# Komputerowe-Projektowanie-Lekow/pmarlo

Hardware: AMD Instinct MI355X
Metric: frames/sec featurize->TICA->k-means->T-matrix, 1Mx64 synth; ITS rel-err (higher is better)
Workload: dtype f64; 1 GPU; synthetic 1000000 frames x 64 f32 features per GPU (AR(1) latents), TICA->10, k=500 (10 Lloyd iterations), lag=10, row-normalised T; frames_per_gpu=1000000, features=64, tica_dim=10, k=500, lag=10, kmeans_iters=10, parallelism=shards1

## Files before the change

include/msmhip.h:

```cpp
#ifndef MSMHIP_H
#define MSMHIP_H

#include <stddef.h>
#include <stdint.h>

#ifdef __cplusplus
extern "C" {
#endif

typedef struct msm_ctx msm_ctx;
typedef struct msm_event msm_event;
typedef struct msm_graph msm_graph;

typedef enum {
    MSM_OK = 0,
    MSM_ERR_INVALID = 1,
    MSM_ERR_HIP = 2,
    MSM_ERR_NOMEM = 3,
    MSM_ERR_UNSUPPORTED = 4,
    MSM_ERR_NOCONV = 5
} msm_status;

typedef enum { MSM_F32 = 0, MSM_F64 = 1 } msm_dtype;

// ... 100 lines not shown
msm_status msm_lagged_moments_onesided(msm_ctx* ctx, const void* d_x, msm_dtype dtype, int64_t n, int F,
                                       int64_t ld, const int64_t* h_seg_start, const int64_t* h_seg_stop,
                                       int n_seg, int lag, const double* d_shift, int assume_finite,
                                       double* d_moments);

msm_status msm_onesided_tica_eigenvalues(msm_ctx* ctx, const double* d_moments, int F, double clip,
                                         double* d_eigvals);

msm_status msm_moments_from_lagged(msm_ctx* ctx, const void* d_x, msm_dtype dtype, int64_t n, int F, int64_t ld,
                                   const int64_t* h_seg_start, const int64_t* h_seg_stop, int n_seg, int lag,
                                   const double* d_shift, const double* d_moments, double* d_sums);

msm_status msm_tica_solve(msm_ctx* ctx, const double* d_moments, const double* d_scale, int F,
                          double epsilon, int kinetic_map, double* d_eigvals, double* d_coeffs,
                          double* d_mean, int* d_rank);

msm_status msm_project(msm_ctx* ctx, const void* d_x, msm_dtype dtype, int64_t n, int F, int64_t ld,
                       const double* d_mu, const double* d_inv_sigma, const double* d_mean2,
                       const double* d_w, int d, int64_t ldw, double* d_y, int64_t ldy, double* d_absmax);

msm_status msm_project_finite(msm_ctx* ctx, const void* d_x, msm_dtype dtype, int64_t n, int F, int64_t ld,
                              const double* d_mu, const double* d_inv_sigma, const double* d_mean2,
                              const double* d_w, int d, int64_t ldw, double* d_y, int64_t ldy, double* d_absmax);

msm_status msm_eigh(msm_ctx* ctx, const double* d_a, int n, double* d_w, double* d_v, int* d_sweeps);

msm_status msm_autocorr_lagscan(msm_ctx* ctx, const void* d_x, msm_dtype dtype, int64_t n, int F, int64_t ld,
                                const int64_t* h_seg_start, const int64_t* h_seg_stop, int n_seg,
                                const int32_t* h_lags, int n_lag, double var_floor, double* d_value,
                                int32_t* d_nvalid);
// ... 212 lines not shown
```

pmarlo_amd/_lib.py:

```python

from __future__ import annotations

import ctypes as C
from pathlib import Path

__all__ = ["lib", "load", "LIB_PATH", "check", "MsmError", "DECLARED_SYMBOLS"]

LIB_PATH = Path(__file__).resolve().parent / "csrc" / "libmsmhip.so"

MSM_OK, MSM_ERR_INVALID, MSM_ERR_HIP, MSM_ERR_NOMEM, MSM_ERR_UNSUPPORTED, MSM_ERR_NOCONV = range(6)
MSM_F32, MSM_F64 = 0, 1
SUPERPOSE_TILE_FRAMES, SUPERPOSE_TILE_FLOATS, SUPERPOSE_LDS_ATOMS, SUPERPOSE_NARROW_SEL = 64, 12288, 4096, 64
REP_MAX_D, REP_GROUP_CHUNK, REP_TILE_I, REP_TILE_J = 256, 1024, 128, 64
REP_FLAG_NONFINITE, REP_FLAG_NEGATIVE, REP_FLAG_NONPOSITIVE_SUM = 1, 2, 4
REP_SCORE_CENTROID, REP_SCORE_MEDOID = 0, 1
REP_SELECT_SMALLEST, REP_SELECT_DIVERSE = 0, 1
SIL_SEG_LEN, SIL_TILE_I = 1024, 128
COMBINE_MAX_SEG, FLUX_LDS_MAX_N = 32, 127


class MsmError(RuntimeError):
    """A HIP-side failure reported through the C ABI."""


# ... 34 lines not shown
    "msm_hbond_presence": (_i32, [_vp, _vp, _i64, _i32, _vp, _i32, C.c_float, C.c_float, _vp]),
    "msm_dssp": (_i32, [_vp, _vp, _i64, _i32, _vp, _vp, _vp, _i32, _vp]),
    "msm_superpose": (_i32, [_vp, _vp, _i64, _i32, _vp, _i32, _vp, _vp, _vp]),
    "msm_count_transitions": (_i32, [_vp, _vp, _i64, _vp, _vp, _i32, _i32, _i32, _i32, _vp, _vp]),
    "msm_count_transitions_weighted": (
        _i32, [_vp, _vp, _vp, _i64, _vp, _vp, _i32, _i32, _i32, _i32, _vp, _vp]),
    "msm_count_transitions_lagscan": (_i32, [_vp, _vp, _i64, _vp, _vp, _i32, _vp, _i32, _i32, _vp, _vp]),
    "msm_state_counts": (_i32, [_vp, _vp, _i64, _i32, _vp]),
    "msm_column_moments_partial": (_i32, [_vp, _vp, _i32, _i64, _i32, _i64, _vp, _vp, _vp]),
    "msm_moments_finalize": (_i32, [_vp, _vp, _vp, _i32, _i32, _vp, _vp, _vp]),
    "msm_column_moments": (_i32, [_vp, _vp, _i32, _i64, _i32, _i64, _i32, _vp, _vp, _vp]),
    "msm_column_minmax": (_i32, [_vp, _vp, _i32, _i64, _i32, _i64, _vp, _vp, _vp]),
    "msm_standardise_params": (_i32, [_vp, _vp, _vp, _i32, _f64, _i32, _vp, _vp, _vp]),
    "msm_lagged_moments": (_i32, [_vp, _vp, _i32, _i64, _i32, _i64, _vp, _vp, _i32, _i32, _vp, _i32, _vp]),
    "msm_tica_solve": (_i32, [_vp, _vp, _vp, _i32, _f64, _i32, _vp, _vp, _vp, _vp]),
    "msm_lagged_moments_reversible": (_i32, [_vp, _vp, _i32, _i64, _i32, _i64, _vp, _vp, _i32, _i32, _vp, _i32, _vp]),
    "msm_lagged_moments_onesided": (_i32, [_vp, _vp, _i32, _i64, _i32, _i64, _vp, _vp, _i32, _i32, _vp, _i32, _vp]),
    "msm_onesided_tica_eigenvalues": (_i32, [_vp, _vp, _i32, _f64, _vp]),
    "msm_moments_from_lagged": (_i32, [_vp, _vp, _i32, _i64, _i32, _i64, _vp, _vp, _i32, _i32, _vp, _vp, _vp]),
    "msm_project": (_i32, [_vp, _vp, _i32, _i64, _i32, _i64, _vp, _vp, _vp, _vp, _i32, _i64, _vp, _i64, _vp]),
    "msm_project_finite": (_i32, [_vp, _vp, _i32, _i64, _i32, _i64, _vp, _vp, _vp, _vp, _i32, _i64, _vp, _i64, _vp]),
    "msm_eigh": (_i32, [_vp, _vp, _i32, _vp, _vp, _vp]),
    "msm_autocorr_lagscan": (_i32, [_vp, _vp, _i32, _i64, _i32, _i64, _vp, _vp, _i32, _vp, _i32, _f64, _vp, _vp]),
    "msm_hstack_f64": (_i32, [_vp, _vp, _i32, _i32, _i64, _vp, _i32, _i32, _i64, _i64, _vp]),
    "msm_kmeans_assign": (_i32, [_vp, _vp, _i32, _i64, _i32, _i64, _vp, _i32, _vp, _vp, _vp, _vp]),
    "msm_kmeans_fit": (_i32, [_vp, _vp, _i32, _i64, _i32, _i64, _vp, _vp, _i32, C.c_uint64, _i32, _i32, _f64, _vp, _vp]),
    "msm_kmeans_fit_begin": (
        _i32, [_vp, _vp, _i32, _i64, _i32, _i64, _vp, _vp, _i32, C.c_uint64, _i32, _f64, _f64, _vp, _vp, _i32]),
    "msm_kmeans_accumulate": (_i32, [_vp, _vp, _i32, _i64, _i32, _i64, _vp, _i32, _vp, _vp, _vp, _vp, _vp]),
    "msm_kmeans_update": (_i32, [_vp, _vp, _vp, _i32, _i32, _vp, _vp, _i32]),
# ... 121 lines not shown
```

pmarlo_amd/csrc/eig.hip:

```cpp
#include "common.h"
#include "wave.h"

__device__ __forceinline__ unsigned long long stamp_clock() {
    unsigned long long t;
    asm volatile("s_memtime %0\n\ts_waitcnt lgkmcnt(0)" : "=s"(t)::"memory");
    return t;
}
#define STAMP_ADD(slot, last) do { const unsigned long long t__ = stamp_clock(); slot += t__ - last; last = t__; } while (0)
#ifdef MSM_JACOBI_STAMPS
__device__ unsigned long long g_jacobi_stamps[8];
#define JSTAMP(i) STAMP_ADD(acc__[i], last__)
#define JSTAMP_INIT unsigned long long acc__[8] = {0, 0, 0, 0, 0, 0, 0, 0}; unsigned long long last__ = stamp_clock();
#define JSTAMP_FLUSH if (threadIdx.x == 0) { for (int i__ = 0; i__ < 8; ++i__) g_jacobi_stamps[i__] += acc__[i__]; }
#else
#define JSTAMP(i)
#define JSTAMP_INIT
#define JSTAMP_FLUSH
#endif
#ifdef MSM_TRI_STAMPS
__device__ unsigned long long g_tri_stamps[24];
#define TSTAMP(i) do { if (threadIdx.x == 0) STAMP_ADD(g_tri_stamps[i], tlast__); } while (0)
#define TSTAMP_INIT unsigned long long tlast__ = 0; if (threadIdx.x == 0) tlast__ = stamp_clock();
#define KSTAMP(i) do { if (threadIdx.x == 0) STAMP_ADD(g_tri_stamps[i], klast__); } while (0)
#define KSTAMP_INIT unsigned long long klast__ = 0; if (threadIdx.x == 0) klast__ = stamp_clock();
// ... 678 lines not shown
        for (int t = 0; t < 8; ++t)
            if (lane == sub + 8 * t && lane < n) ts->inv[lane] = nr_rsqrt(m[t]);
    }
    __syncthreads();
    if (what == 1 && in) {
#pragma unroll
        for (int t = 0; t < 8; ++t) {
            const int i = sub + 8 * t;
            if (i < n) W[lane * ld + i] = m[t] * ts->inv[i];
        }
    }
    __syncthreads();
    return true;
}

__device__ __forceinline__ bool tridiag_eigh(double* A, double* Q, double* X, int n, int ld, TriShared* ts, double orth_tol) {
    const int tid = threadIdx.x, nt = blockDim.x, lane = tid & 63, wave = tid >> 6;
    if (n == 1) {
        if (tid == 0) { ts->lam[0] = A[0]; A[0] = 1.0; }
        __syncthreads();
        return true;
    }
    if (ld != kTriLd) return false;
    TSTAMP_INIT
    if (tid == 0) ts->bad = 0;
    __syncthreads();
    TSTAMP(0);
    householder_phase(A, Q, n, ts);
    TSTAMP(1);
    __syncthreads();
    TSTAMP(2);
    {
// ... 14 lines not shown
            else ts->de[lane] = make_double2(8.0, 0.0);
            if (lane < 8) ts->de[kTriMax + lane] = make_double2(8.0, 0.0);
            if (lane == 0) {
                if (!(an < 1e300)) ts->bad = 1;
                ts->scale = sc;
                const double bn = fmax(fabs(gl), fabs(gu));
                const double pad = 4.0 * n * 2.220446049250313e-16 * bn + 1e-290;
                ts->gl = gl - pad;
                ts->gu = gu + pad;
            }
        }
    }
    __syncthreads();
    TSTAMP(3);
    if (ts->bad) return false;
    if (tid < 8 * kTriMax && wave * 8 < n) {
        const int i = tid >> 3, t = tid & 7;
        const int nblocks = (n + 7) >> 3;
        double lo = ts->gl, hi = ts->gu;
        const double frac = (double)(t + 1) * (1.0 / 9.0);
        for (int it = 0; it < 20; ++it) {
            const double x = fma(hi - lo, frac, lo);
            const int c = sturm_count(ts, nblocks, x);
            double nlo = c <= i ? x : lo, nhi = c > i ? x : hi;
            lo = row8_reduce(nlo, hw_max_f64);
            hi = row8_reduce(nhi, hw_min_f64);
        }
        if (i < n && t == 0) ts->lam[i] = 0.5 * (lo + hi);
    }
    __syncthreads();
    TSTAMP(4);
    const double tiny = 1e-290;
    double* Xc = X + (lane < n ? lane : 0);
    double* Ac = A + (lane < n ? lane : 0);
    const double lamb = ts->lam[lane < n ? lane : 0];
    if (wave == 0 && lane < n) {
        double q = ts->de[0].x - lamb;
        Xc[0] = q;
        for (int j0 = 1; j0 < n; j0 += 8) {
            double2 r[8];
#pragma unroll
            for (int u = 0; u < 8; ++u) r[u] = ts->de[j0 + u];
#pragma unroll
            for (int u = 0; u < 8; ++u) {
                if (j0 + u < n) {
                    if (fabs(q) < tiny) q = -tiny;
                    q = fma(-r[u].y, nr_rcp(q), r[u].x - lamb);
                    Xc[(j0 + u) * ld] = q;
                }
            }
        }
    } else if (wave == 1 && lane < n) {
        double r = ts->de[n - 1].x - lamb;
        if (fabs(r) < tiny) r = -tiny;
        double ir = nr_rcp(r);
        Ac[(n - 1) * ld] = ir;
        for (int j0 = n - 2; j0 >= 0; j0 -= 8) {
            double dj[8], e2[8];
#pragma unroll
            for (int u = 0; u < 8; ++u) {
                const int j = j0 - u >= 0 ? j0 - u : 0;
                dj[u] = ts->de[j].x;
                e2[u] = ts->de[j + 1].y;
            }
#pragma unroll
            for (int u = 0; u < 8; ++u) {
                if (j0 - u >= 0) {
                    r = fma(-e2[u], ir, dj[u] - lamb);
                    if (fabs(r) < tiny) r = -tiny;
                    ir = nr_rcp(r);
                    Ac[(j0 - u) * ld] = ir;
                }
            }
        }
    }
    __syncthreads();
    int kk = n - 1;
    if (wave < 2 && lane < n) {
        double gbest = fabs(Xc[(n - 1) * ld]);
        for (int j0 = n - 2; j0 >= 0; j0 -= 8) {
            double g[8];
#pragma unroll
            for (int u = 0; u < 8; ++u) {
                const int j = j0 - u >= 0 ? j0 - u : 0;
                g[u] = fabs(fma(-ts->de[j + 1].y, Ac[(j + 1) * ld], Xc[j * ld]));
            }
#pragma unroll
            for (int u = 0; u < 8; ++u)
                if (j0 - u >= 0 && g[u] <= gbest) { gbest = g[u]; kk = j0 - u; }
        }
    }
    __syncthreads();
    if (wave == 0 && lane < n) {
        double z = 1.0, nrm2 = 1.0;
        for (int j0 = n - 2; j0 >= 0; j0 -= 8) {
            double f[8];
#pragma unroll
            for (int u = 0; u < 8; ++u) {
                const int j = j0 - u >= 0 ? j0 - u : 0;
                double qq = Xc[j * ld];
                if (fabs(qq) < tiny) qq = -tiny;
                f[u] = -(ts->e[j] * nr_rcp(qq));
            }
#pragma unroll
            for (int u = 0; u < 8; ++u) {
                if (j0 - u >= 0 && j0 - u < kk) {
                    z = f[u] * z;
                    Xc[(j0 - u) * ld] = z;
                    nrm2 = fma(z, z, nrm2);
                }
            }
        }
        Xc[kk * ld] = 1.0;
        ts->praw[lane] = nrm2;
    } else if (wave == 1 && lane < n) {
        double z = 1.0, nrm2 = 0.0;
        for (int j0 = 0; j0 + 1 < n; j0 += 8) {
            double f[8];
#pragma unroll
            for (int u = 0; u < 8; ++u) {
                const int j = j0 + u + 1 < n ? j0 + u : 0;
                f[u] = -(ts->e[j] * Ac[(j + 1) * ld]);
            }
#pragma unroll
            for (int u = 0; u < 8; ++u) {
                if (j0 + u + 1 < n && j0 + u >= kk) {
                    z = f[u] * z;
                    Xc[(j0 + u + 1) * ld] = z;
                    nrm2 = fma(z, z, nrm2);
                }
            }
        }
        ts->uq[lane] = nrm2;
    }
    __syncthreads();
    if (tid < n) {
        const double nrm2 = ts->praw[tid] + ts->uq[tid];
        const bool ok = nrm2 > 0.0 && nrm2 < 1e300;
        ts->inv[tid] = nr_rsqrt(ok ? nrm2 : 1.0);
        if (!ok) ts->bad = 1;
    }
    __syncthreads();
    TSTAMP(5);
    {
        double worst = 0.0;
        bool bad = false;
        for (int e0 = tid; e0 < n * n; e0 += nt) {
            const int j = e0 / n, i = e0 - j * n;
            const double x0 = X[j * ld + i];
            const double xm = j > 0 ? ts->e[j - 1] * X[(j - 1) * ld + i] : 0.0;
            const double xp = j + 1 < n ? ts->e[j] * X[(j + 1) * ld + i] : 0.0;
            const double tx = fma(ts->d[j] - ts->lam[i], x0, xm + xp) * ts->inv[i];
            bad = bad || !(fabs(tx) <= 1e-10);
        }
        const int jj = lane & 15, g = lane >> 4;
        const int tiles = (n + 15) >> 4;
        for (int t = wave; t < tiles * tiles; t += nt >> 6) {
            const int a0 = (t / tiles) * 16, b0 = (t - (t / tiles) * tiles) * 16;
            if (b0 > a0) continue;
            const bool aok = a0 + jj < n, bok = b0 + jj < n;
            const int ai = aok ? a0 + jj : 0, bi = bok ? b0 + jj : 0;
            const double sa = ts->inv[ai], sb = ts->inv[bi];
            const tri_v4f64 acc = mfma_tile_acc(
                n, g, aok, bok, [&](int k) { return X[k * ld + ai] * sa; }, [&](int k) { return X[k * ld + bi] * sb; });
#pragma unroll
            for (int r = 0; r < 4; ++r) {
                const int row = a0 + g + 4 * r, col = b0 + jj;
                if (row < n && col < n) worst = fmax(worst, fabs(acc[r] - (row == col ? 1.0 : 0.0)));
            }
        }
        if (bad) worst = 1e300;
#pragma unroll
        for (int off = 32; off > 0; off >>= 1) worst = fmax(worst, __shfl_xor(worst, off, 64));
        if (lane == 0) ts->red[wave] = worst;
        __syncthreads();
        worst = 0.0;
        for (int w = 0; w < nt / 64; ++w) worst = fmax(worst, ts->red[w]);
        TSTAMP(6);
        if (ts->bad || !(worst <= orth_tol)) return false;
    }
    mfma_mm<true, false>(A, Q, X, n, n, n, ld, ts->inv);
    if (tid < n) ts->lam[tid] /= ts->scale;
    __syncthreads();
    TSTAMP(7);
    return true;
}

__device__ __forceinline__ int eigh_with_fallback(double* A, double* V, double* X, int n, int ld, double* backup,
                                                  bool try_tri, TriShared* ts, JacobiShared* sh, double orth_tol,
                                                  double* ev_out, const double*& vec) {
    const int tid = threadIdx.x, nt = blockDim.x;
    if (try_tri) {
        for (int e = tid; e < n * n; e += nt) backup[e] = A[(e / n) * ld + (e % n)];
        __syncthreads();
        if (tridiag_eigh(A, V, X, n, ld, ts, orth_tol)) {
            for (int i = tid; i < n; i += nt) ev_out[i] = ts->lam[i];
            vec = A;
            return 0;
        }
        __syncthreads();
        for (int e = tid; e < n * n; e += nt) A[(e / n) * ld + (e % n)] = backup[e];
        __syncthreads();
    }
    const int sweeps = jacobi_eigh(A, V, n, ld, sh, 40);
    for (int i = tid; i < n; i += nt) ev_out[i] = A[i * ld + i];
    vec = V;
    return sweeps;
}

struct TicaWork {
    double *A, *V, *B1, *B2, *ev, *mean, *isc;
    int* order;
};

template <int lds_mats>
__global__ __launch_bounds__(kEigThreads) void tica_solve_kernel(
    const double* __restrict__ mom, const double* __restrict__ scale, int n, int ld, double epsilon, int kinetic_map,
    TicaWork wk, double* __restrict__ out_eig, double* __restrict__ out_W, double* __restrict__ out_mean,
    int* __restrict__ out_rank) {
    extern __shared__ __attribute__((aligned(16))) unsigned char smem_raw[];
    __shared__ JacobiShared sh;
    __shared__ TriShared ts;
    const int tid = threadIdx.x, nt = blockDim.x;
    double* lds = reinterpret_cast<double*>(smem_raw);
    const size_t mat = (size_t)n * ld;
    double *A, *V, *B1, *B2;
    if constexpr (lds_mats >= 2) { A = lds; V = lds + mat; } else { A = wk.A; V = wk.V; }
    if constexpr (lds_mats >= 4) { B1 = lds + 2 * mat; B2 = lds + 3 * mat; } else { B1 = wk.B1; B2 = wk.B2; }

    const double* M00 = mom;
    const double* M0t = mom + (size_t)n * n;
    const double* sx = M0t + (size_t)n * n;
    const double* sy = sx + n;
// ... 97 lines not shown
        canonical_signs(B2, n, rank, ld);
        for (int e = tid; e < n * rank; e += nt) {
            const int i = e / rank, j = e - i * rank;
            B2[i * ld + j] /= sqrt(wk.ev[wk.order[j]]);
        }
        __syncthreads();
    }
    mfma_mm<false, false>(A, B1, B2, n, rank, n, ld);
    mfma_mm<true, false>(V, B2, A, rank, rank, n, ld);
    for (int e = tid; e < rank * rank; e += nt) {
        const int i = e / rank, j = e - i * rank;
        A[i * ld + j] = 0.5 * (V[i * ld + j] + V[j * ld + i]);
    }
    __syncthreads();
    KSTAMP(10);
    const double* Vec;
    eigh_with_fallback(A, V, B1, rank, ld, wk.A, kFused && rank <= kTriMax, &ts, &sh, 1e-11, wk.ev, Vec);
    __syncthreads();
    KSTAMP(11);
    if (kFused && n <= kTriMax) {
        double* evl = ts.praw;
        double* sgn = ts.uq;
        int* ord = sh.p;
        if (tid < rank) evl[tid] = wk.ev[tid];
        __syncthreads();
        rank_order<true>(rank, ord, [&](int i) { return fabs(evl[i]); });
        mfma_mm<false, false>(B1, B2, Vec, n, rank, rank, ld);
        {
            const int lane = tid & 63, wave = tid >> 6;
            for (int j = wave; j < rank; j += nt >> 6) {
                double best = lane < n ? fabs(B1[lane * ld + j]) : -1.0;
                int bi = lane;
                double val = lane < n ? B1[lane * ld + j] : 0.0;
                wave_argmax_xor(best, bi, val);
                if (lane == 0) sgn[j] = val < 0.0 ? -1.0 : 1.0;
            }
        }
        __syncthreads();
        for (int e = tid; e < n * n; e += nt) {
            const int i = e / n, j = e - i * n;
            double v = 0.0;
            if (j < rank) {
                const int c = ord[j];
                v = B1[i * ld + c] * sgn[c];
                if (kinetic_map) v *= evl[c];
            }
            out_W[e] = v;
        }
        for (int j = tid; j < n; j += nt) out_eig[j] = j < rank ? evl[ord[j]] : 0.0;
        KSTAMP(12);
        return;
    }
    sort_desc_abs(wk.ev, rank, wk.order);
    mfma_mm<false, false>(B1, B2, Vec, n, rank, rank, ld);
    canonical_signs(B1, n, rank, ld);
    for (int e = tid; e < n * n; e += nt) {
        const int i = e / n, j = e - i * n;
        double v = 0.0;
        if (j < rank) {
            v = B1[i * ld + wk.order[j]];
            if (kinetic_map) v *= wk.ev[wk.order[j]];
        }
        out_W[e] = v;
    }
    for (int j = tid; j < n; j += nt) out_eig[j] = j < rank ? wk.ev[wk.order[j]] : 0.0;
    KSTAMP(12);
}

template <bool use_lds>
__global__ __launch_bounds__(kEigThreads) void eigh_kernel(const double* __restrict__ Ain, int n, int ld,
                                                          double* gA, double* gV, int* order,
                                                          double* __restrict__ out_w, double* __restrict__ out_v,
                                                          int* __restrict__ out_sweeps) {
    extern __shared__ __attribute__((aligned(16))) unsigned char smem_raw[];
    __shared__ JacobiShared sh;
    __shared__ TriShared ts;
    const int tid = threadIdx.x, nt = blockDim.x;
    double *A, *V;
    if constexpr (use_lds) { A = reinterpret_cast<double*>(smem_raw); V = A + (size_t)n * ld; }
    else { A = gA; V = gV; }
    for (int e = tid; e < n * n; e += nt) {
        const int i = e / n, j = e - i * n;
        A[i * ld + j] = 0.5 * (Ain[e] + Ain[j * n + i]);
    }
    __syncthreads();
    const double* vec;
    const int sweeps = eigh_with_fallback(A, V, V + (size_t)n * ld, n, ld, gA, use_lds && n <= kTriMax, &ts, &sh, 1e-12,
                                          out_w, vec);
    if (vec == A) {
        if (out_v)
            for (int e = tid; e < n * n; e += nt) out_v[e] = A[(e / n) * ld + (e % n)];
        if (tid == 0 && out_sweeps) *out_sweeps = 0;
        return;
    }
    rank_order<false>(n, order, [&](int i) { return A[i * ld + i]; });
    __syncthreads();
    for (int j = tid; j < n; j += nt) out_w[j] = A[order[j] * ld + order[j]];
    if (out_v)
        for (int e = tid; e < n * n; e += nt) {
            const int i = e / n, j = e - i * n;
            out_v[e] = V[i * ld + order[j]];
        }
    if (tid == 0 && out_sweeps) *out_sweeps = sweeps;
// ... 16 lines not shown
    const double* sy = sx + n;
    const double T = sy[n];
    if (!(T > 0.0)) {
        for (int i = tid; i < n; i += nt) out_eig[i] = 0.0;
        return;
    }
    const double den = T - 1.0 > 1.0 ? T - 1.0 : 1.0;
    for (int e = tid; e < n * n; e += nt) {
        const int i = e / n, j = e - i * n;
        const double c0 = 0.5 * (M00[e] + M00[j * n + i]) - sx[i] * sx[j] / T;
        P0[i * ld + j] = c0 / den;
        P1[i * ld + j] = (M0t[e] - sx[i] * sy[j] / T) / den;
    }
    __syncthreads();
    auto eigh = [&](const double*& vec) {
        eigh_with_fallback(P0, P2, P3, n, ld, gbak, use_lds && n <= kTriMax, &ts, &sh, 1e-12, gw, vec);
        __syncthreads();
    };
    const double* vec = nullptr;
    eigh(vec);
    for (int e = tid; e < n * n; e += nt) {
        const int i = e / n, j = e - i * n;
        const double wj = gw[j] > clip ? gw[j] : clip;
        P3[i * ld + j] = vec[i * ld + j] / sqrt(sqrt(wj));
    }
    __syncthreads();
    mfma_mm<false, true>(P0, P3, P3, n, n, n, ld);
    mfma_mm<false, false>(P2, P0, P1, n, n, n, ld);
    mfma_mm<false, false>(P3, P2, P0, n, n, n, ld);
    for (int e = tid; e < n * n; e += nt) {
        const int i = e / n, j = e - i * n;
// ... 21 lines not shown
template <typename... Params, typename... Args>
msm_status launch_single_workgroup(msm_ctx* ctx, void (*kern)(Params...), size_t lds_bytes, Args... args) {
    if (lds_bytes > 48 * 1024)
        MSM_HIP(ctx, hipFuncSetAttribute((const void*)kern, hipFuncAttributeMaxDynamicSharedMemorySize, (int)lds_bytes));
    hipLaunchKernelGGL(kern, dim3(1), dim3(kEigThreads), lds_bytes, ctx->stream, args...);
    MSM_CHECK_LAUNCH(ctx);
    return MSM_OK;
}

}

extern "C" {

msm_status msm_tica_solve(msm_ctx* ctx, const double* d_moments, const double* d_scale, int F, double epsilon,
                          int kinetic_map, double* d_eigvals, double* d_coeffs, double* d_mean, int* d_rank) {
    if (!ctx) return MSM_ERR_INVALID;
    MSM_REQUIRE(ctx, F >= 1 && F <= 2 * kMaxPairs, "msm_tica_solve: need 1 <= F <= %d (got %d)", 2 * kMaxPairs, F);
    MSM_REQUIRE(ctx, epsilon >= 0.0, "msm_tica_solve: epsilon must be >= 0");
    MSM_REQUIRE(ctx, d_moments && d_eigvals && d_coeffs && d_mean && d_rank, "msm_tica_solve: NULL pointer");
    const int ld = eig_ld(F);
    const size_t mat = (size_t)F * ld;
    const size_t need = (4 * mat + 3 * F) * sizeof(double) + (size_t)F * sizeof(int) + 64;
    msm_status rs = msm_reserve_scratch(ctx, need);
    if (rs != MSM_OK) return rs;
    double* base = (double*)ctx->scratch;
    TicaWork wk;
    wk.A = base; wk.V = base + mat; wk.B1 = base + 2 * mat; wk.B2 = base + 3 * mat;
    wk.ev = base + 4 * mat; wk.mean = wk.ev + F; wk.isc = wk.mean + F; wk.order = (int*)(wk.isc + F);
    const size_t lds_budget = 150 * 1024;
    int lds_mats = 0;
    if (4 * mat * sizeof(double) <= lds_cap(lds_budget, kStaticLdsTri)) lds_mats = 4;
    else if (2 * mat * sizeof(double) <= lds_cap(lds_budget, kStaticLdsJacobi)) lds_mats = 2;
    const size_t lds = (size_t)lds_mats * mat * sizeof(double);
    auto kern = lds_mats == 4 ? tica_solve_kernel<4> : (lds_mats == 2 ? tica_solve_kernel<2> : tica_solve_kernel<0>);
    return launch_single_workgroup(ctx, kern, lds, d_moments, d_scale, F, ld, epsilon, kinetic_map, wk, d_eigvals, d_coeffs,
                                   d_mean, d_rank);
}

msm_status msm_onesided_tica_eigenvalues(msm_ctx* ctx, const double* d_moments, int F, double clip, double* d_eigvals) {
    if (!ctx) return MSM_ERR_INVALID;
    MSM_REQUIRE(ctx, F >= 1 && F <= 2 * kMaxPairs, "msm_onesided_tica_eigenvalues: need 1 <= F <= %d (got %d)",
                2 * kMaxPairs, F);
    MSM_REQUIRE(ctx, d_moments && d_eigvals && clip > 0.0, "msm_onesided_tica_eigenvalues: bad arguments");
    const int ld = eig_ld(F);
    const size_t mat = (size_t)F * ld;
    const size_t lds = 4 * mat * sizeof(double);
    const bool use_lds = lds <= lds_cap(140 * 1024, kStaticLdsTri);
    msm_status rs = msm_reserve_scratch(ctx, ((use_lds ? 0 : 4 * mat) + (size_t)F * F + F) * sizeof(double) +
                                                 (size_t)F * sizeof(int) + 64);
    if (rs != MSM_OK) return rs;
    double* gP = (double*)ctx->scratch;
// ... 26 lines not shown
```

pmarlo_amd/device.py:

```python

from __future__ import annotations

import ctypes as C
import os
import sys
from typing import Iterable, Sequence

import numpy as np

from . import _lib
from ._lib import check, lib

__all__ = ["Engine", "DeviceArray", "get_engine", "segments_to_bounds"]


def _dtype_code(dtype: np.dtype) -> int:
    dtype = np.dtype(dtype)
    if dtype == np.float32:
        return _lib.MSM_F32
    if dtype == np.float64:
        return _lib.MSM_F64
    raise TypeError(f"feature matrices must be float32 or float64, got {dtype}")


# ... 487 lines not shown
        return out

    def moments_from_lagged(self, x: DeviceArray, lag: int, shift: DeviceArray, moments: DeviceArray, *, starts=None,
                            stops=None, out: DeviceArray | None = None, ld: int | None = None) -> DeviceArray:
        n, F = x.shape
        if starts is None:
            starts, stops = segments_to_bounds(None, n)
        starts, stops = self._seg_ptrs(starts, stops)
        out = out if out is not None else self.empty((3 * F,), np.float64)
        check(lib.msm_moments_from_lagged(self.handle, x.ptr, _dtype_code(x.dtype), n, F, int(F if ld is None else ld),
                                          starts.ctypes.data, stops.ctypes.data, len(starts), int(lag), shift.ptr,
                                          moments.ptr, out.ptr), self.handle)
        return out

    def tica_solve(self, moments: DeviceArray, F: int, *, scale: DeviceArray | None = None,
                   epsilon: float = 1e-6, kinetic_map: bool = True, out=None):
        if out is not None:
            eig, W, mean, rank = out
        else:
            eig = self.empty((F,), np.float64)
            W = self.empty((F, F), np.float64)
            mean = self.empty((F,), np.float64)
            rank = self.empty((1,), np.int32)
        check(lib.msm_tica_solve(self.handle, moments.ptr, scale.ptr if scale is not None else None, F,
                                 float(epsilon), int(bool(kinetic_map)), eig.ptr, W.ptr, mean.ptr, rank.ptr),
              self.handle)
        return eig, W, mean, rank

    def project(self, x: DeviceArray, mu: DeviceArray, inv_sigma: DeviceArray, W: DeviceArray, d: int, *,
                mean2: DeviceArray | None = None, out: DeviceArray | None = None,
                absmax: DeviceArray | None = None, assume_finite: bool = False, ld: int | None = None) -> DeviceArray:
        n, F = x.shape
        ldw = W.shape[1]
        out = out if out is not None else self.empty((n, d), np.float64)
        fn = lib.msm_project_finite if assume_finite else lib.msm_project
        check(fn(self.handle, x.ptr, _dtype_code(x.dtype), n, F, int(F if ld is None else ld), mu.ptr, inv_sigma.ptr,
                 mean2.ptr if mean2 is not None else None, W.ptr, int(d), ldw, out.ptr,
                 out.shape[1], absmax.ptr if absmax is not None else None), self.handle)
        return out

    def eigh(self, a: DeviceArray, want_vectors: bool = True):
# ... 722 lines not shown
```

pmarlo_amd/dist.py:

```python

from __future__ import annotations

import ctypes as C
import os
import time
from dataclasses import dataclass
from pathlib import Path

import numpy as np

from .device import DeviceArray, Engine

__all__ = ["Comm", "NativeComm", "TorchComm", "ShardedMSM", "ShardConfig", "exchange_shapes", "exchange_aliases",
           "torch_exchange_buffers", "bootstrap_id"]


class Comm:

    world = 1
    rank = 0

    def allreduce_sum(self, name: str) -> None: ...
    def allreduce_sum_from(self, name: str, src) -> None: ...
    def allreduce_min(self, name: str) -> None: ...
# ... 272 lines not shown
                raise ValueError("ShardConfig.pairs must list n_features atom pairs")
            self.xyz = x
            self.pairs_d = eng.to_device(np.ascontiguousarray(cfg.pairs, np.int32).reshape(F, 2))
            self.x = eng.empty((n, F), np.float32)
            eng.featurize_distances_into(self.xyz, self.pairs_d, self.x)
        else:
            self.xyz = None
            self.x = x
        if cfg.tica_dim > 0:
            self.mean, self.scale, self.inv_scale = (eng.empty((F,), np.float64) for _ in range(3))
            self.eig = eng.empty((F,), np.float64)
            self.W = eng.empty((F, F), np.float64)
            self.m2 = eng.empty((F,), np.float64)
            self.rank_d = eng.empty((1,), np.int32)
            self.Y = eng.empty((n, d), np.float64)
        else:
            self.Y = self.x
        self.labels = eng.empty((n,), np.int32)
        self.T = eng.empty((k, k), np.float64)
        self.rowsum = eng.empty((k,), np.float64)
        self.diag = eng.empty((1,), np.float64)
        self.km_sums = b["km_acc"].view((k * d,), np.int64)
        self.km_counts = b["km_acc"].view((k,), np.int64, offset_elems=k * d)
        multi_shard = self.comm is not None and (self.comm.world > 1 or self.always_exchange)
        self.km_local = eng.empty((k * d + k,), np.int64) if multi_shard else None
        nbytes = eng.kmeans_image_bytes(n, d)
        self.km_image = eng.empty((nbytes,), np.uint8) if nbytes else None
        self.accum_events: list = []
        self.stage_events: dict = {}
        self.time_accum = False
# ... 19 lines not shown
        multi = comm is not None and (comm.world > 1 or self.always_exchange)
        F, d, k = cfg.n_features, cfg.cluster_dim, cfg.k
        self._stamp("begin")
        if self.xyz is not None:
            eng.featurize_distances_into(self.xyz, self.pairs_d, self.x)
            self._stamp("featurize")
        if cfg.tica_dim > 0:
            eng.lagged_moments(self.x, cfg.lag, b["shift"], assume_finite=True, out=b["lagged"], symmetric=True)
            eng.moments_from_lagged(self.x, cfg.lag, b["shift"], b["lagged"], out=b["mom_sums"])
            if multi:
                comm.allreduce_sum("moments")
            eng.standardise_params(b["mom_sums"], b["shift"], F, float(self.n_total), True,
                                   out=(self.mean, self.scale, self.inv_scale))
            self._stamp("moments")
            eng.tica_solve(b["lagged"], F, scale=self.scale, epsilon=1e-6, kinetic_map=True,
                           out=(self.eig, self.W, self.m2, self.rank_d))
            self._stamp("tica_solve")
            eng.project(self.x, b["shift"], self.inv_scale, self.W, d, mean2=self.m2, out=self.Y,
                        absmax=b["fit_state"].view((1,), offset_elems=2), assume_finite=True)
            self._stamp("project")
        eng.kmeans_fit_begin(self.Y, k, seed=cfg.seed, n_total=self.n_total, tol2=0.0, centers=b["centers"],
                             state=b["fit_state"], absmax_ready=cfg.tica_dim > 0)
        if multi:
            if comm.rank != 0:
                b["centers"].fill_bytes_(0x7F)
            b["start_scale"].copy_from(b["fit_scale"])
            comm.allreduce_min("start")
            b["fit_scale"].copy_from(b["start_scale"])
            comm.reciprocal("fit_inv_scale", "fit_scale")
        acc = self.km_local if self.km_local is not None else b["km_acc"]
        acc.zero_()
# ... 57 lines not shown
```

pmarlo_amd/markov_state_model/reduction.py:

```python

from __future__ import annotations

from typing import Optional, List, Sequence

import numpy as np

from ..device import get_engine
from ..pipeline import MSMPipeline, TicaModel

__all__ = ["tica_reduce", "pca_reduce", "vamp_reduce", "reduce_features", "tica_fit_transform_trajectories",
           "preprocess_params"]


def _as_matrix(X) -> np.ndarray:
    X = np.asarray(X)
    if X.dtype not in (np.float32, np.float64):
        X = X.astype(np.float64)
    if X.ndim == 1:
        X = X.reshape(-1, 1)
    if X.ndim != 2:
        raise ValueError(f"Expected 2D array, got shape {X.shape}")
    return np.ascontiguousarray(X)


# ... 173 lines not shown
                                    lag: int) -> tuple[np.ndarray, TicaModel]:
    n_components = int(max(2, min(5, n_components_hint)))
    drop = int(max(0, lag or 0))
    lag = int(max(1, lag or 1))
    Xm = _as_matrix(features)
    edges = np.concatenate([[0], np.cumsum([int(v) for v in traj_lengths])])
    if edges[-1] != Xm.shape[0]:
        raise ValueError("trajectory lengths do not add up to the number of feature rows")
    segs = [(int(a), int(b)) for a, b in zip(edges[:-1], edges[1:])]
    eng = get_engine()
    pipe = MSMPipeline(eng)
    xd = eng.to_device(Xm)
    mu, _, _, has_nan = pipe.standardise_params(xd, scale=False)
    one = eng.to_device(np.ones(Xm.shape[1]))
    mom = pipe.tica_moments(xd, lag, mu, segments=segs, assume_finite=not has_nan, symmetric=True)
    model = pipe.tica_solve(mom, mu, one, one, lag, n_components)
    model.dim = min(n_components, int(model.rank.to_host()[0]))
    Y = pipe.tica_transform(model, xd, assume_finite=not has_nan).to_host()
    keep: List[np.ndarray] = []
    for a, b in segs:
        keep.append(Y[a:b - drop] if b - a > drop else np.empty((0, Y.shape[1])))
    return (np.vstack(keep) if keep else Y), model
```

pmarlo_amd/pipeline.py:

```python

from __future__ import annotations

from dataclasses import dataclass, field
from typing import Sequence

import numpy as np

from .device import DeviceArray, Engine, segments_to_bounds

__all__ = ["TicaModel", "MSMPipeline", "PipelineResult"]

_EPS_SCALE = 10 * np.finfo(float).eps


@dataclass
class TicaModel:

    mu: DeviceArray
    sigma: DeviceArray
    inv_sigma: DeviceArray
    eigenvalues: DeviceArray
    coefficients: DeviceArray
    mean: DeviceArray
    rank: DeviceArray
# ... 40 lines not shown
                                           symmetric=symmetric)
        total = None
        for i in range(0, len(starts), 16):
            part = self.eng.lagged_moments(x, lag, mu, starts=starts[i:i + 16], stops=stops[i:i + 16],
                                           assume_finite=assume_finite, symmetric=symmetric).to_host()
            total = part if total is None else total + part
        return self.eng.to_device(total) if out is None else out.copy_from_host(total)

    def tica_fit(self, x: DeviceArray, lag: int, dim: int, *, scale: bool = True, segments=None,
                 epsilon: float = 1e-6, kinetic_map: bool = True) -> TicaModel:
        mu, sigma, inv_sigma, has_nan = self.standardise_params(x, scale=scale)
        mom = self.tica_moments(x, lag, mu, segments=segments, assume_finite=not has_nan, symmetric=True)
        return self.tica_solve(mom, mu, sigma, inv_sigma, lag, dim, epsilon=epsilon, kinetic_map=kinetic_map)

    def tica_solve(self, moments: DeviceArray, mu, sigma, inv_sigma, lag: int, dim: int, *, epsilon: float = 1e-6,
                   kinetic_map: bool = True) -> TicaModel:
        F = mu.shape[0]
        eig, W, mean, rank = self.eng.tica_solve(moments, F, scale=sigma, epsilon=epsilon, kinetic_map=kinetic_map)
        return TicaModel(mu, sigma, inv_sigma, eig, W, mean, rank, int(lag), int(dim), moments)

    def tica_transform(self, model: TicaModel, x: DeviceArray, out: DeviceArray | None = None,
                       assume_finite: bool = False) -> DeviceArray:
        return self.eng.project(x, model.mu, model.inv_sigma, model.coefficients, model.dim, mean2=model.mean, out=out,
                                assume_finite=assume_finite)

    def cluster(self, y: DeviceArray, k: int, *, seed: int = 0, max_iter: int = 50, tol: float = 1e-4,
                whiten: tuple[DeviceArray, DeviceArray] | None = None, centers: DeviceArray | None = None,
                labels: DeviceArray | None = None, mindist: DeviceArray | None = None, fit: bool = True):
        eng = self.eng
        mean, std = whiten if whiten is not None else (None, None)
        state = None
        if fit:
            n, d = y.shape
# ... 37 lines not shown
```

Before: 715.9 million frames/s.

## Compute only leading TICA eigenpairs in tridiagonal eigensolver

Adds a leading-eigenpair mode to the tridiagonal eigensolver. It bisects only for eigenvalues at both spectrum ends, picks the top tica_dim by magnitude, and computes eigenvectors and back-transforms only for those candidates. It falls back to the full solve when the candidates are not well separated. The aim is to cut single-workgroup eigen-solve work inside TICA, which is a tiny part of a pipeline dominated by 1M-frame passes, at the cost of extra branching and a guard-based fallback.

```diff
diff --git a/include/msmhip.h b/include/msmhip.h
--- a/include/msmhip.h
+++ b/include/msmhip.h
@@ -138,6 +138,10 @@
 msm_status msm_tica_solve(msm_ctx* ctx, const double* d_moments, const double* d_scale, int F,
                           double epsilon, int kinetic_map, double* d_eigvals, double* d_coeffs,
                           double* d_mean, int* d_rank);
+
+msm_status msm_tica_solve_leading(msm_ctx* ctx, const double* d_moments, const double* d_scale, int F,
+                                  double epsilon, int kinetic_map, double* d_eigvals, double* d_coeffs,
+                                  double* d_mean, int* d_rank, int n_lead);
 
 msm_status msm_project(msm_ctx* ctx, const void* d_x, msm_dtype dtype, int64_t n, int F, int64_t ld,
                        const double* d_mu, const double* d_inv_sigma, const double* d_mean2,
diff --git a/pmarlo_amd/_lib.py b/pmarlo_amd/_lib.py
--- a/pmarlo_amd/_lib.py
+++ b/pmarlo_amd/_lib.py
@@ -72,6 +72,7 @@
     "msm_standardise_params": (_i32, [_vp, _vp, _vp, _i32, _f64, _i32, _vp, _vp, _vp]),
     "msm_lagged_moments": (_i32, [_vp, _vp, _i32, _i64, _i32, _i64, _vp, _vp, _i32, _i32, _vp, _i32, _vp]),
     "msm_tica_solve": (_i32, [_vp, _vp, _vp, _i32, _f64, _i32, _vp, _vp, _vp, _vp]),
+    "msm_tica_solve_leading": (_i32, [_vp, _vp, _vp, _i32, _f64, _i32, _vp, _vp, _vp, _vp, _i32]),
     "msm_lagged_moments_reversible": (_i32, [_vp, _vp, _i32, _i64, _i32, _i64, _vp, _vp, _i32, _i32, _vp, _i32, _vp]),
     "msm_lagged_moments_onesided": (_i32, [_vp, _vp, _i32, _i64, _i32, _i64, _vp, _vp, _i32, _i32, _vp, _i32, _vp]),
     "msm_onesided_tica_eigenvalues": (_i32, [_vp, _vp, _i32, _f64, _vp]),
diff --git a/pmarlo_amd/csrc/eig.hip b/pmarlo_amd/csrc/eig.hip
--- a/pmarlo_amd/csrc/eig.hip
+++ b/pmarlo_amd/csrc/eig.hip
@@ -716,8 +716,11 @@
     return true;
 }
 
-__device__ __forceinline__ bool tridiag_eigh(double* A, double* Q, double* X, int n, int ld, TriShared* ts, double orth_tol) {
+constexpr double kTriGuard = 1e-6;
+__device__ __forceinline__ bool tridiag_eigh(double* A, double* Q, double* X, int n, int ld, TriShared* ts, double orth_tol,
+                                             int want, int* sel, int& kept) {
     const int tid = threadIdx.x, nt = blockDim.x, lane = tid & 63, wave = tid >> 6;
+    kept = 0;
     if (n == 1) {
         if (tid == 0) { ts->lam[0] = A[0]; A[0] = 1.0; }
         __syncthreads();
@@ -762,27 +765,52 @@
     __syncthreads();
     TSTAMP(3);
     if (ts->bad) return false;
-    if (tid < 8 * kTriMax && wave * 8 < n) {
-        const int i = tid >> 3, t = tid & 7;
-        const int nblocks = (n + 7) >> 3;
-        double lo = ts->gl, hi = ts->gu;
-        const double frac = (double)(t + 1) * (1.0 / 9.0);
-        for (int it = 0; it < 20; ++it) {
-            const double x = fma(hi - lo, frac, lo);
-            const int c = sturm_count(ts, nblocks, x);
-            double nlo = c <= i ? x : lo, nhi = c > i ? x : hi;
-            lo = row8_reduce(nlo, hw_max_f64);
-            hi = row8_reduce(nhi, hw_min_f64);
-        }
-        if (i < n && t == 0) ts->lam[i] = 0.5 * (lo + hi);
-    }
-    __syncthreads();
+    bool lead = want > 0 && 2 * (want + 2) < n;
+    int nb = lead ? 2 * (want + 2) : n;
+    int na = n;
+    for (;;) {
+        if (tid < 8 * kTriMax && wave * 8 < nb) {
+            const int b = tid >> 3, t = tid & 7;
+            const int i = !lead || b < want + 2 ? b : n - nb + b;
+            const int nblocks = (n + 7) >> 3;
+            double lo = ts->gl, hi = ts->gu;
+            const double frac = (double)(t + 1) * (1.0 / 9.0);
+            for (int it = 0; it < 20; ++it) {
+                const double x = fma(hi - lo, frac, lo);
+                const int c = sturm_count(ts, nblocks, x);
+                double nlo = c <= i ? x : lo, nhi = c > i ? x : hi;
+                lo = row8_reduce(nlo, hw_max_f64);
+                hi = row8_reduce(nhi, hw_min_f64);
+            }
+            if (b < nb && t == 0) ts->lam[i] = 0.5 * (lo + hi);
+        }
+        __syncthreads();
+        if (!lead) break;
+        const int nc = 2 * (want + 1);
+        const auto cand = [&](int c) { return c <= want ? c : n - nc + c; };
+        const auto key = [&](int c) { return fabs(ts->lam[cand(c)] / ts->scale); };
+        rank_order<true>(nc, sel, key);
+        __syncthreads();
+        const bool lone = ts->lam[want + 1] - ts->lam[want] > kTriGuard &&
+                          ts->lam[n - want - 1] - ts->lam[n - want - 2] > kTriGuard;
+        if (lone && key(sel[want - 1]) != key(sel[want])) {
+            const double lk = tid < nc ? ts->lam[cand(tid)] : 0.0;
+            __syncthreads();
+            if (tid < nc) ts->lam[tid] = lk;
+            __syncthreads();
+            na = nc;
+            break;
+        }
+        __syncthreads();
+        lead = false;
+        nb = n;
+    }
     TSTAMP(4);
     const double tiny = 1e-290;
-    double* Xc = X + (lane < n ? lane : 0);
-    double* Ac = A + (lane < n ? lane : 0);
-    const double lamb = ts->lam[lane < n ? lane : 0];
-    if (wave == 0 && lane < n) {
+    double* Xc = X + (lane < na ? lane : 0);
+    double* Ac = A + (lane < na ? lane : 0);
+    const double lamb = ts->lam[lane < na ? lane : 0];
+    if (wave == 0 && lane < na) {
         double q = ts->de[0].x - lamb;
         Xc[0] = q;
         for (int j0 = 1; j0 < n; j0 += 8) {
@@ -798,7 +826,7 @@
                 }
             }
         }
-    } else if (wave == 1 && lane < n) {
+    } else if (wave == 1 && lane < na) {
         double r = ts->de[n - 1].x - lamb;
         if (fabs(r) < tiny) r = -tiny;
         double ir = nr_rcp(r);
@@ -824,7 +852,7 @@
     }
     __syncthreads();
     int kk = n - 1;
-    if (wave < 2 && lane < n) {
+    if (wave < 2 && lane < na) {
         double gbest = fabs(Xc[(n - 1) * ld]);
         for (int j0 = n - 2; j0 >= 0; j0 -= 8) {
             double g[8];
@@ -839,7 +867,7 @@
         }
     }
     __syncthreads();
-    if (wave == 0 && lane < n) {
+    if (wave == 0 && lane < na) {
         double z = 1.0, nrm2 = 1.0;
         for (int j0 = n - 2; j0 >= 0; j0 -= 8) {
             double f[8];
@@ -861,7 +889,7 @@
         }
         Xc[kk * ld] = 1.0;
         ts->praw[lane] = nrm2;
-    } else if (wave == 1 && lane < n) {
+    } else if (wave == 1 && lane < na) {
         double z = 1.0, nrm2 = 0.0;
         for (int j0 = 0; j0 + 1 < n; j0 += 8) {
             double f[8];
@@ -882,7 +910,7 @@
         ts->uq[lane] = nrm2;
     }
     __syncthreads();
-    if (tid < n) {
+    if (tid < na) {
         const double nrm2 = ts->praw[tid] + ts->uq[tid];
         const bool ok = nrm2 > 0.0 && nrm2 < 1e300;
         ts->inv[tid] = nr_rsqrt(ok ? nrm2 : 1.0);
@@ -893,8 +921,8 @@
     {
         double worst = 0.0;
         bool bad = false;
-        for (int e0 = tid; e0 < n * n; e0 += nt) {
-            const int j = e0 / n, i = e0 - j * n;
+        for (int e0 = tid; e0 < n * na; e0 += nt) {
+            const int j = e0 / na, i = e0 - j * na;
             const double x0 = X[j * ld + i];
             const double xm = j > 0 ? ts->e[j - 1] * X[(j - 1) * ld + i] : 0.0;
             const double xp = j + 1 < n ? ts->e[j] * X[(j + 1) * ld + i] : 0.0;
@@ -902,11 +930,11 @@
             bad = bad || !(fabs(tx) <= 1e-10);
         }
         const int jj = lane & 15, g = lane >> 4;
-        const int tiles = (n + 15) >> 4;
+        const int tiles = (na + 15) >> 4;
         for (int t = wave; t < tiles * tiles; t += nt >> 6) {
             const int a0 = (t / tiles) * 16, b0 = (t - (t / tiles) * tiles) * 16;
             if (b0 > a0) continue;
-            const bool aok = a0 + jj < n, bok = b0 + jj < n;
+            const bool aok = a0 + jj < na, bok = b0 + jj < na;
             const int ai = aok ? a0 + jj : 0, bi = bok ? b0 + jj : 0;
             const double sa = ts->inv[ai], sb = ts->inv[bi];
             const tri_v4f64 acc = mfma_tile_acc(
@@ -914,7 +942,7 @@
 #pragma unroll
             for (int r = 0; r < 4; ++r) {
                 const int row = a0 + g + 4 * r, col = b0 + jj;
-                if (row < n && col < n) worst = fmax(worst, fabs(acc[r] - (row == col ? 1.0 : 0.0)));
+                if (row < na && col < na) worst = fmax(worst, fabs(acc[r] - (row == col ? 1.0 : 0.0)));
             }
         }
         if (bad) worst = 1e300;
@@ -927,25 +955,28 @@
         TSTAMP(6);
         if (ts->bad || !(worst <= orth_tol)) return false;
     }
-    mfma_mm<true, false>(A, Q, X, n, n, n, ld, ts->inv);
-    if (tid < n) ts->lam[tid] /= ts->scale;
+    mfma_mm<true, false>(A, Q, X, n, na, n, ld, ts->inv);
+    if (tid < na) ts->lam[tid] /= ts->scale;
     __syncthreads();
     TSTAMP(7);
+    kept = na < n ? na : 0;
     return true;
 }
 
 __device__ __forceinline__ int eigh_with_fallback(double* A, double* V, double* X, int n, int ld, double* backup,
                                                   bool try_tri, TriShared* ts, JacobiShared* sh, double orth_tol,
-                                                  double* ev_out, const double*& vec) {
+                                                  double* ev_out, const double*& vec, int want, int& kept) {
     const int tid = threadIdx.x, nt = blockDim.x;
+    kept = 0;
     if (try_tri) {
         for (int e = tid; e < n * n; e += nt) backup[e] = A[(e / n) * ld + (e % n)];
         __syncthreads();
-        if (tridiag_eigh(A, V, X, n, ld, ts, orth_tol)) {
-            for (int i = tid; i < n; i += nt) ev_out[i] = ts->lam[i];
+        if (tridiag_eigh(A, V, X, n, ld, ts, orth_tol, want, sh->p, kept)) {
+            for (int i = tid; i < (kept ? kept : n); i += nt) ev_out[i] = ts->lam[i];
             vec = A;
             return 0;
         }
+        kept = 0;
         __syncthreads();
         for (int e = tid; e < n * n; e += nt) A[(e / n) * ld + (e % n)] = backup[e];
         __syncthreads();
@@ -964,7 +995,7 @@
 template <int lds_mats>
 __global__ __launch_bounds__(kEigThreads) void tica_solve_kernel(
     const double* __restrict__ mom, const double* __restrict__ scale, int n, int ld, double epsilon, int kinetic_map,
-    TicaWork wk, double* __restrict__ out_eig, double* __restrict__ out_W, double* __restrict__ out_mean,
+    int n_lead, TicaWork wk, double* __restrict__ out_eig, double* __restrict__ out_W, double* __restrict__ out_mean,
     int* __restrict__ out_rank) {
     extern __shared__ __attribute__((aligned(16))) unsigned char smem_raw[];
     __shared__ JacobiShared sh;
@@ -1092,21 +1123,26 @@
     }
     __syncthreads();
     KSTAMP(10);
+    const int keep = n_lead > 0 && n_lead < rank ? n_lead : rank;
+    const bool lds_tail = kFused && n <= kTriMax;
     const double* Vec;
-    eigh_with_fallback(A, V, B1, rank, ld, wk.A, kFused && rank <= kTriMax, &ts, &sh, 1e-11, wk.ev, Vec);
+    int kept;
+    eigh_with_fallback(A, V, B1, rank, ld, wk.A, kFused && rank <= kTriMax, &ts, &sh, 1e-11, wk.ev, Vec,
+                       lds_tail && keep < rank ? keep : 0, kept);
     __syncthreads();
     KSTAMP(11);
-    if (kFused && n <= kTriMax) {
+    if (lds_tail) {
         double* evl = ts.praw;
         double* sgn = ts.uq;
         int* ord = sh.p;
-        if (tid < rank) evl[tid] = wk.ev[tid];
-        __syncthreads();
-        rank_order<true>(rank, ord, [&](int i) { return fabs(evl[i]); });
-        mfma_mm<false, false>(B1, B2, Vec, n, rank, rank, ld);
+        const int ncol = kept ? kept : rank;
+        if (tid < ncol) evl[tid] = wk.ev[tid];
+        __syncthreads();
+        rank_order<true>(ncol, ord, [&](int i) { return fabs(evl[i]); });
+        mfma_mm<false, false>(B1, B2, Vec, n, ncol, rank, ld);
         {
             const int lane = tid & 63, wave = tid >> 6;
-            for (int j = wave; j < rank; j += nt >> 6) {
+            for (int j = wave; j < ncol; j += nt >> 6) {
                 double best = lane < n ? fabs(B1[lane * ld + j]) : -1.0;
                 int bi = lane;
                 double val = lane < n ? B1[lane * ld + j] : 0.0;
@@ -1118,14 +1154,14 @@
         for (int e = tid; e < n * n; e += nt) {
             const int i = e / n, j = e - i * n;
             double v = 0.0;
-            if (j < rank) {
+            if (j < keep) {
                 const int c = ord[j];
                 v = B1[i * ld + c] * sgn[c];
                 if (kinetic_map) v *= evl[c];
             }
             out_W[e] = v;
         }
-        for (int j = tid; j < n; j += nt) out_eig[j] = j < rank ? evl[ord[j]] : 0.0;
+        for (int j = tid; j < n; j += nt) out_eig[j] = j < keep ? evl[ord[j]] : 0.0;
         KSTAMP(12);
         return;
     }
@@ -1135,13 +1171,13 @@
     for (int e = tid; e < n * n; e += nt) {
         const int i = e / n, j = e - i * n;
         double v = 0.0;
-        if (j < rank) {
+        if (j < keep) {
             v = B1[i * ld + wk.order[j]];
             if (kinetic_map) v *= wk.ev[wk.order[j]];
         }
         out_W[e] = v;
     }
-    for (int j = tid; j < n; j += nt) out_eig[j] = j < rank ? wk.ev[wk.order[j]] : 0.0;
+    for (int j = tid; j < n; j += nt) out_eig[j] = j < keep ? wk.ev[wk.order[j]] : 0.0;
     KSTAMP(12);
 }
 
@@ -1163,8 +1199,9 @@
     }
     __syncthreads();
     const double* vec;
+    int kept;
     const int sweeps = eigh_with_fallback(A, V, V + (size_t)n * ld, n, ld, gA, use_lds && n <= kTriMax, &ts, &sh, 1e-12,
-                                          out_w, vec);
+                                          out_w, vec, 0, kept);
     if (vec == A) {
         if (out_v)
             for (int e = tid; e < n * n; e += nt) out_v[e] = A[(e / n) * ld + (e % n)];
@@ -1211,7 +1248,8 @@
     }
     __syncthreads();
     auto eigh = [&](const double*& vec) {
-        eigh_with_fallback(P0, P2, P3, n, ld, gbak, use_lds && n <= kTriMax, &ts, &sh, 1e-12, gw, vec);
+        int kept;
+        eigh_with_fallback(P0, P2, P3, n, ld, gbak, use_lds && n <= kTriMax, &ts, &sh, 1e-12, gw, vec, 0, kept);
         __syncthreads();
     };
     const double* vec = nullptr;
@@ -1263,6 +1301,12 @@
 
 msm_status msm_tica_solve(msm_ctx* ctx, const double* d_moments, const double* d_scale, int F, double epsilon,
                           int kinetic_map, double* d_eigvals, double* d_coeffs, double* d_mean, int* d_rank) {
+    return msm_tica_solve_leading(ctx, d_moments, d_scale, F, epsilon, kinetic_map, d_eigvals, d_coeffs, d_mean, d_rank, 0);
+}
+
+msm_status msm_tica_solve_leading(msm_ctx* ctx, const double* d_moments, const double* d_scale, int F, double epsilon,
+                                  int kinetic_map, double* d_eigvals, double* d_coeffs, double* d_mean, int* d_rank,
+                                  int n_lead) {
     if (!ctx) return MSM_ERR_INVALID;
     MSM_REQUIRE(ctx, F >= 1 && F <= 2 * kMaxPairs, "msm_tica_solve: need 1 <= F <= %d (got %d)", 2 * kMaxPairs, F);
     MSM_REQUIRE(ctx, epsilon >= 0.0, "msm_tica_solve: epsilon must be >= 0");
@@ -1282,8 +1326,8 @@
     else if (2 * mat * sizeof(double) <= lds_cap(lds_budget, kStaticLdsJacobi)) lds_mats = 2;
     const size_t lds = (size_t)lds_mats * mat * sizeof(double);
     auto kern = lds_mats == 4 ? tica_solve_kernel<4> : (lds_mats == 2 ? tica_solve_kernel<2> : tica_solve_kernel<0>);
-    return launch_single_workgroup(ctx, kern, lds, d_moments, d_scale, F, ld, epsilon, kinetic_map, wk, d_eigvals, d_coeffs,
-                                   d_mean, d_rank);
+    return launch_single_workgroup(ctx, kern, lds, d_moments, d_scale, F, ld, epsilon, kinetic_map,
+                                   n_lead > 0 && n_lead < F ? n_lead : 0, wk, d_eigvals, d_coeffs, d_mean, d_rank);
 }
 
 msm_status msm_onesided_tica_eigenvalues(msm_ctx* ctx, const double* d_moments, int F, double clip, double* d_eigvals) {
diff --git a/pmarlo_amd/device.py b/pmarlo_amd/device.py
--- a/pmarlo_amd/device.py
+++ b/pmarlo_amd/device.py
@@ -525,7 +525,7 @@
         return out
 
     def tica_solve(self, moments: DeviceArray, F: int, *, scale: DeviceArray | None = None,
-                   epsilon: float = 1e-6, kinetic_map: bool = True, out=None):
+                   epsilon: float = 1e-6, kinetic_map: bool = True, out=None, n_lead: int = 0):
         if out is not None:
             eig, W, mean, rank = out
         else:
@@ -533,9 +533,9 @@
             W = self.empty((F, F), np.float64)
             mean = self.empty((F,), np.float64)
             rank = self.empty((1,), np.int32)
-        check(lib.msm_tica_solve(self.handle, moments.ptr, scale.ptr if scale is not None else None, F,
-                                 float(epsilon), int(bool(kinetic_map)), eig.ptr, W.ptr, mean.ptr, rank.ptr),
-              self.handle)
+        check(lib.msm_tica_solve_leading(self.handle, moments.ptr, scale.ptr if scale is not None else None, F,
+                                         float(epsilon), int(bool(kinetic_map)), eig.ptr, W.ptr, mean.ptr, rank.ptr,
+                                         int(n_lead)), self.handle)
         return eig, W, mean, rank
 
     def project(self, x: DeviceArray, mu: DeviceArray, inv_sigma: DeviceArray, W: DeviceArray, d: int, *,
diff --git a/pmarlo_amd/dist.py b/pmarlo_amd/dist.py
--- a/pmarlo_amd/dist.py
+++ b/pmarlo_amd/dist.py
@@ -2,6 +2,7 @@
 from __future__ import annotations
 
 import ctypes as C
+import inspect
 import os
 import time
 from dataclasses import dataclass
@@ -310,6 +311,8 @@
             self.m2 = eng.empty((F,), np.float64)
             self.rank_d = eng.empty((1,), np.int32)
             self.Y = eng.empty((n, d), np.float64)
+            can_lead = "n_lead" in inspect.signature(eng.tica_solve).parameters
+            self._lead_kw = {"n_lead": int(cfg.tica_dim)} if can_lead else {}
         else:
             self.Y = self.x
         self.labels = eng.empty((n,), np.int32)
@@ -359,7 +362,7 @@
                                    out=(self.mean, self.scale, self.inv_scale))
             self._stamp("moments")
             eng.tica_solve(b["lagged"], F, scale=self.scale, epsilon=1e-6, kinetic_map=True,
-                           out=(self.eig, self.W, self.m2, self.rank_d))
+                           out=(self.eig, self.W, self.m2, self.rank_d), **self._lead_kw)
             self._stamp("tica_solve")
             eng.project(self.x, b["shift"], self.inv_scale, self.W, d, mean2=self.m2, out=self.Y,
                         absmax=b["fit_state"].view((1,), offset_elems=2), assume_finite=True)
diff --git a/pmarlo_amd/markov_state_model/reduction.py b/pmarlo_amd/markov_state_model/reduction.py
--- a/pmarlo_amd/markov_state_model/reduction.py
+++ b/pmarlo_amd/markov_state_model/reduction.py
@@ -211,7 +211,7 @@
     mu, _, _, has_nan = pipe.standardise_params(xd, scale=False)
     one = eng.to_device(np.ones(Xm.shape[1]))
     mom = pipe.tica_moments(xd, lag, mu, segments=segs, assume_finite=not has_nan, symmetric=True)
-    model = pipe.tica_solve(mom, mu, one, one, lag, n_components)
+    model = pipe.tica_solve(mom, mu, one, one, lag, n_components, all_pairs=True)
     model.dim = min(n_components, int(model.rank.to_host()[0]))
     Y = pipe.tica_transform(model, xd, assume_finite=not has_nan).to_host()
     keep: List[np.ndarray] = []
diff --git a/pmarlo_amd/pipeline.py b/pmarlo_amd/pipeline.py
--- a/pmarlo_amd/pipeline.py
+++ b/pmarlo_amd/pipeline.py
@@ -78,9 +78,10 @@
         return self.tica_solve(mom, mu, sigma, inv_sigma, lag, dim, epsilon=epsilon, kinetic_map=kinetic_map)
 
     def tica_solve(self, moments: DeviceArray, mu, sigma, inv_sigma, lag: int, dim: int, *, epsilon: float = 1e-6,
-                   kinetic_map: bool = True) -> TicaModel:
+                   kinetic_map: bool = True, all_pairs: bool = False) -> TicaModel:
         F = mu.shape[0]
-        eig, W, mean, rank = self.eng.tica_solve(moments, F, scale=sigma, epsilon=epsilon, kinetic_map=kinetic_map)
+        eig, W, mean, rank = self.eng.tica_solve(moments, F, scale=sigma, epsilon=epsilon, kinetic_map=kinetic_map,
+                                                 n_lead=0 if all_pairs else int(dim))
         return TicaModel(mu, sigma, inv_sigma, eig, W, mean, rank, int(lag), int(dim), moments)
 
     def tica_transform(self, model: TicaModel, x: DeviceArray, out: DeviceArray | None = None,
```

Result: faster. 726.0 million frames/s (median of 6 runs) (+1.4%).
